# kaiidams/Kokoro-Align

Hardware: NVIDIA B200
Metric: lattice cells/sec (TxS) (higher is better)
Workload: dtype f32

## Files before the change

kokoro-align_b200/csrc/kab_api.cu:

```cuda
#include "../../include/kokoro_align_b200.h"

#include <algorithm>
#include <atomic>
#include <chrono>
#include <map>
#include <mutex>
#include <thread>
#include <unordered_map>
#include <cstdio>
#include <cstdlib>
#include <cstring>
#include <limits>
#include <new>
#include <vector>

#include "kab_band.cuh"
#include "kab_bandp.cuh"
#include "kab_bandr.cuh"
#include "kab_btpar.cuh"
#include "kab_wide.cuh"
#include "kab_common.cuh"
#include "kab_compact.cuh"
#include "kab_debug.h"
#include "kab_generic.cuh"
// ... 316 lines not shown
      if (mask && !mask[b]) continue;
      const int64_t T = t_off[b + 1] - t_off[b], S = 2 * (l_off[b + 1] - l_off[b]) + 1;
      if (band_shaped(T, S)) { any_band = true; ok = std::min<int64_t>(W, S) <= ga_max_weff; }
    }
    pl->band_ga = ok && any_band;
  }
  if (!ctc && V > MAX_STAGE_V && M <= 4) {
    std::vector<uint8_t> seen((size_t)V, 0);
    int64_t dmax = 0;
    bool any = false;
    for (int64_t b = 0; b < B; ++b) {
      if (mask && !mask[b]) continue;
      const int64_t L = l_off[b + 1] - l_off[b];
      const int32_t *lab = labels + l_off[b];
      if (pl->band_ga && band_shaped(t_off[b + 1] - t_off[b], 2 * L + 1)) continue;
      bool usable = true;
      int64_t dist = 0;
      for (int64_t l = 0; l < L && usable; ++l) {
        if (lab[l] <= 0 || lab[l] >= V) usable = false;
        else if (!seen[(size_t)lab[l]]) { seen[(size_t)lab[l]] = 1; ++dist; }
      }
      for (int64_t l = 0; l < L; ++l)
        if (lab[l] > 0 && lab[l] < V) seen[(size_t)lab[l]] = 0;
      if (usable) { dmax = std::max(dmax, dist); any = true; }
    }
    if (any && dmax + 1 <= MAX_STAGE_V) {
      pl->Vc = (int32_t)std::max<int64_t>(8, align_up(dmax + 1, 4));
      h_gather.assign((size_t)B * pl->Vc, 0);
    }
  }
  const int32_t Veff = pl->Vc ? pl->Vc : V;

  pl->stage_frames = Veff <= 64 ? 16 : 8;
  if (const char *sf = getenv("KAB_STAGE_FRAMES")) {
    const int v = atoi(sf);
    if (v == 8 || v == 16 || v == 32) pl->stage_frames = v;
  }
  pl->stage_bytes = (int32_t)align_up((int64_t)pl->stage_frames * Veff * 4 + 24, 16);

  int wide_capacity = 0;
  {
    const KabWideGeom wgeo = kab_wide_geom(pl->stage_bytes);
    int occ = 0;
    if (wgeo.smem_bytes <= 227 * 1024 &&
        ensure_dyn_smem((const void *)kab_wide_kernel, device, wgeo.smem_bytes) == cudaSuccess &&
        cudaOccupancyMaxActiveBlocksPerMultiprocessor(&occ, kab_wide_kernel, KAB_WD_THREADS, wgeo.smem_bytes) == cudaSuccess)
      wide_capacity = occ * pl->sm_count;
    (void)cudaGetLastError();
  }
  int wide_max_ctas = 0;

  std::vector<uint16_t> col16;
  std::vector<int32_t> status_init((size_t)B, 0);
  int64_t bp_bytes = 0, scr_floats = 0, max_band_weff = 0;
  std::vector<uint8_t> hyb_mask;
  int hyb_k = 0;
  kab_plan_info &info = pl->info;
  info.n_lattices = B; info.device = device; info.total_frames = pl->total_T;
  const int n_mask = (V + 63) / 64;
  struct LatFacts { uint8_t bad, special, compact; int32_t distinct; int64_t col_off; };
  std::vector<LatFacts> facts((size_t)B);
  auto for_lattices = [&](auto &&fn) {
    const unsigned hw = std::thread::hardware_concurrency();
    const int nt = (B >= 2048 && pl->total_L >= 65536 && hw >= 4 && !getenv("KAB_SERIAL_SETUP")) ? (int)std::min<unsigned>(8, hw / 2) : 1;
    auto work = [&](int t) {
      std::vector<int64_t> words((size_t)std::max(n_mask, 1), 0);
      const int64_t b0 = B * t / nt, b1 = B * (t + 1) / nt;
      for (int64_t b = b0; b < b1; ++b)
        if (!mask || mask[b]) fn(b, words.data());
    };
    std::vector<std::thread> th;
    for (int t = 1; t < nt; ++t) th.emplace_back(work, t);
    work(0);
    for (auto &x : th) x.join();
  };
  for_lattices([&](int64_t b, int64_t *distinct_mask) {
    const int64_t T = t_off[b + 1] - t_off[b], L = l_off[b + 1] - l_off[b], S = 2 * L + 1;
    const int32_t *lab = labels + l_off[b];
    LatFacts f{};
    std::fill(distinct_mask, distinct_mask + n_mask, (int64_t)0);
    for (int64_t l = 0; l < L; ++l) {
      if (ctc ? (lab[l] < 0 || lab[l] >= V || lab[l] == blank) : (lab[l] < -V || lab[l] >= V)) { f.bad = 1; break; }
      if (!ctc && lab[l] <= 0) f.special = 1;
      const int32_t c = lab[l] < 0 ? lab[l] + V : lab[l];
      if (!(distinct_mask[c >> 6] >> (c & 63) & 1)) { distinct_mask[c >> 6] |= (int64_t)1 << (c & 63); ++f.distinct; }
    }
    const bool ga = pl->band_ga && !f.special && band_shaped(T, S);
    if (!f.bad && pl->Vc && !f.special && !ga && f.distinct + 1 <= pl->Vc) {
      f.compact = 1;
      int32_t *g = h_gather.data() + (size_t)b * pl->Vc;
      int32_t n = 1;
      for (int w = 0; w < n_mask; ++w)
        for (int64_t m = distinct_mask[w]; m; m &= m - 1) g[n++] = w * 64 + __builtin_ctzll((unsigned long long)m);
    }
    facts[(size_t)b] = f;
  });
  {
    int64_t off = 0;
    for (int64_t b = 0; b < B; ++b) {
      if (mask && !mask[b]) continue;
      facts[(size_t)b].col_off = off;
      if (!facts[(size_t)b].bad) off += align_up(l_off[b + 1] - l_off[b], 8) + 8;
    }
    col16.assign((size_t)off, 0);
  }
  for_lattices([&](int64_t b, int64_t *) {
    const LatFacts &f = facts[(size_t)b];
    if (f.bad) return;
    const int64_t L = l_off[b + 1] - l_off[b];
    const int32_t *lab = labels + l_off[b];
    uint16_t *c = col16.data() + f.col_off;
    if (f.compact) {
      const int32_t *g = h_gather.data() + (size_t)b * pl->Vc;
      const int32_t n = f.distinct + 1;
      for (int64_t l = 0; l < L; ++l) c[l] = (uint16_t)(std::lower_bound(g + 1, g + n, lab[l]) - g);
    } else {
      for (int64_t l = 0; l < L; ++l) c[l] = (uint16_t)(lab[l] < 0 ? lab[l] + V : lab[l]);
    }
  });
  for (int64_t b = 0; b < B; ++b) {
    if (mask && !mask[b]) continue;
    const int64_t T = t_off[b + 1] - t_off[b], L = l_off[b + 1] - l_off[b], S = 2 * L + 1;
    const bool bad = facts[(size_t)b].bad != 0, special = facts[(size_t)b].special != 0;
    const int64_t distinct = facts[(size_t)b].distinct;
    if (bad) {
      status_init[(size_t)b] = KAB_ST_BAD_LABEL;
      pl->any_bad_label = true;
      continue;
    }
    if (ctc) {
      const int32_t *lab = labels + l_off[b];
      int64_t R = 0;
      for (int64_t l = 1; l < L; ++l) R += lab[l] == lab[l - 1];
      if (T < L + R) {
        status_init[(size_t)b] = KAB_ST_DEAD_BAND;
        pl->any_bad_label = true;
        continue;
      }
    }
    KabLattice d{};
    d.t_off = t_off[b];
    d.lab_off = l_off[b];
    d.T = (int32_t)T; d.L = (int32_t)L; d.index = (int32_t)b;
    d.col_off = facts[(size_t)b].col_off;
    const bool ga = pl->band_ga && !special && band_shaped(T, S);

    const bool fast = M <= 4 && !special && (ga || (Veff <= MAX_STAGE_V && (!pl->Vc || distinct + 1 <= pl->Vc)));
    const bool full = W >= S && (S * (T - 1)) / T <= W / 2;
    const int64_t weff = ctc ? S : std::min<int64_t>(W, S);
    int q;
    if (fast && !ga && full && S <= 248) {
      q = Q_WARP;
      d.k = S <= 62 ? 2 : (S <= 124 ? 4 : (S <= 186 ? 6 : 8));
      const int fpw = d.k <= 2 ? 8 : (d.k <= 4 ? 4 : 2);
      d.bp_off = bp_bytes;
      bp_bytes += align_up((T + fpw - 1) / fpw * 128, 256);
    } else if (fast && W >= 1 && S <= 3 * T && weff + 32 <= KAB_BAND_OW * BAND_MAX_WARPS) {
      q = Q_BAND;
      max_band_weff = std::max(max_band_weff, weff);
    } else if (fast && !ga && M == 4 && full && ((S + KAB_BAND_OW - 1) / KAB_BAND_OW + KAB_WD_CW - 1) / KAB_WD_CW + 1 <= wide_capacity) {
      q = Q_WIDE;
      const int nww = (int)((S + KAB_BAND_OW - 1) / KAB_BAND_OW);
      d.k = nww;
      wide_max_ctas = std::max(wide_max_ctas, (nww + KAB_WD_CW - 1) / KAB_WD_CW);
      d.bp_off = bp_bytes;
      bp_bytes += (int64_t)nww * ((T + 7) / 8) * 256;
      d.scr_off = pl->wide_ws_bytes / 4;
      pl->wide_ws_bytes += (int64_t)align_up((int64_t)kab_wide_ws_bytes(nww), 256);
    } else {
      q = Q_GENERIC;
      d.bp_off = bp_bytes;
      bp_bytes += align_up(T * std::max<int64_t>(1, weff), 256);
      d.scr_off = scr_floats;
      scr_floats += align_up(2 * (S + 16), 64);
    }
    pl->lists[q].push_back(d);
    pl->max_T[q] = std::max(pl->max_T[q], (int)T);
    info.n_class[q == Q_WARP ? KAB_CLASS_WARP : (q == Q_GENERIC ? KAB_CLASS_GENERIC : (q == Q_WIDE ? KAB_CLASS_WIDE : KAB_CLASS_BAND))]++;
    const int64_t cells = ctc ? T * S : cells_eval_of(T, S, W);
    info.cells_eval += cells;
    info.cells_nominal += T * S;
    int bbits = 0;
    while ((1 << bbits) < M) ++bbits;
    const int64_t dcols = std::min<int64_t>(V, distinct + 1);
    info.algorithmic_bytes += 4 * dcols * T + (cells * bbits + 7) / 8 + (T * bbits + 7) / 8 + 12 * T;
  }
  if (!pl->lists[Q_BAND].empty()) {
    pl->band_nw = (int32_t)((max_band_weff + 32 + KAB_BAND_OW - 1) / KAB_BAND_OW);
    const int nc = (pl->band_nw + KAB_BP_CW - 1) / KAB_BP_CW;
    const char *cl = getenv("KAB_BAND_CLUSTER");
    int want_nc = cl ? atoi(cl) : -1;
    if (band_mode >= 0) want_nc = band_mode == 0 ? 0 : -1;
    const bool cluster_ok = nc <= 8 && kab_bandp_geom(pl->stage_bytes).smem_bytes <= 227 * 1024;
    const int nwq = (int)((max_band_weff + 32 + KAB_BQ_OW - 1) / KAB_BQ_OW);
    const int ncq = (nwq + KAB_BQ_CW - 1) / KAB_BQ_CW;
    const bool q_ok = ncq <= 8 && kab_bandq_geom(pl->stage_bytes).smem_bytes <= 227 * 1024;
    const int ncr = (nwq + KAB_BR_CW - 1) / KAB_BR_CW;
    const bool r_ok = pl->band_ga || (ncr <= 8 && pl->stage_frames == KAB_BR_F && kab_bandr_geom(pl->stage_bytes).smem_bytes <= 227 * 1024);
    const char *qe = getenv("KAB_BAND_Q");
    const int want_q = band_mode >= 0 ? (band_mode == 0 ? 0 : -1) : (qe ? atoi(qe) : -1);
    const char *re = getenv("KAB_BAND_R");
    const int want_r = band_mode >= 0 ? band_mode : (re ? atoi(re) : -1);
    int64_t n_band = (int64_t)pl->lists[Q_BAND].size();
    double sum_t = 0.0, max_t = 0.0, bt_steps = 0.0;
    for (const KabLattice &d : pl->lists[Q_BAND]) {
      sum_t += d.T; max_t = std::max(max_t, (double)d.T);
      bt_steps += (double)d.T * (double)std::min<int64_t>(W, 2 * (int64_t)d.L + 1);
    }
    const double est_r = std::max(max_t * 70.0, sum_t / std::max(1, pl->sm_count / std::max(1, ncr)) * 90.0) + bt_steps * 0.55e-3;
    const double est_b = std::max(max_t, sum_t / (double)(pl->sm_count * (pl->band_nw <= 16 ? 2 : 1))) * 190.0;
    const bool use_r = pl->band_ga || (r_ok && want_r != 0 && want_nc != 0 && want_q != 0 && (want_r >= 1 || want_nc >= 1 || est_r <= est_b));
    const bool use_q = !use_r && M == 4 && q_ok && want_q != 0 && want_nc != 0 && (want_q >= 1 || n_band <= pl->sm_count / ncq);
    {
      const char *he = getenv("KAB_BAND_HYBRID");
      const int want_h = he ? atoi(he) : -1;
      if (band_mode < 0 && !mask && !use_r && !use_q && r_ok && !pl->band_ga && !pl->Vc && V <= MAX_STAGE_V && want_h != 0 &&
          want_r < 0 && want_q < 0 && want_nc < 0 && n_band >= 2) {
        std::vector<KabLattice> &bl = pl->lists[Q_BAND];
        std::stable_sort(bl.begin(), bl.end(), [](const KabLattice &a, const KabLattice &b2) { return a.T > b2.T; });
        std::vector<double> pre((size_t)n_band + 1, 0.0);
        for (int64_t i = 0; i < n_band; ++i) pre[(size_t)i + 1] = pre[(size_t)i] + bl[(size_t)i].T;
        const int per_sm = pl->band_nw <= 16 ? 2 : 1;
        double best = est_b;
        int best_k = 0;
        int64_t best_m = 0;
        for (int k = 1; k <= pl->sm_count / ncr / 2; ++k) {
          const double sm_left = (double)(pl->sm_count - k * ncr) * per_sm;
          for (int64_t m = k; m < n_band && m <= 16 * (int64_t)k; ++m) {
            const double tr_ = std::max((double)bl[0].T, pre[(size_t)m] / k) * 70.0;
            const double tb_ = std::max((double)bl[(size_t)m].T, (sum_t - pre[(size_t)m]) / sm_left) * 190.0;
            const double ms = std::max(tr_, tb_);
            if (ms < best) { best = ms; best_k = k; best_m = m; }
          }
        }
        if (want_h >= 1 && best_k == 0) { best_k = 1; best_m = 1; }
        if (best_k > 0 && (want_h >= 1 || best < 0.85 * est_b)) {
          hyb_mask.assign((size_t)B, 0);
          for (int64_t i = 0; i < best_m; ++i) hyb_mask[(size_t)bl[(size_t)i].index] = 1;
          bl.erase(bl.begin(), bl.begin() + best_m);
          hyb_k = best_k;
          want_nc = 0;
          pl->band_sm_reserved = best_k * ncr;
          n_band = (int64_t)bl.size();
          pl->max_T[Q_BAND] = bl.empty() ? 0 : bl[0].T;
        }
      }
    }
    if (use_r || use_q) {
      pl->band_q = true;
      pl->band_r = use_r;
      pl->band_cw = use_r ? KAB_BR_CW : KAB_BQ_CW;
      pl->band_nc = use_r ? ncr : ncq;
      const int nwt = pl->band_cw * pl->band_nc;
      for (KabLattice &d : pl->lists[Q_BAND]) {
        d.bp_off = bp_bytes;
        bp_bytes += (int64_t)((d.T + 7) / 8) * 128 * nwt;
        d.scr_off = pl->band_fifo_bytes / 4;
        pl->band_fifo_bytes += (int64_t)align_up((int64_t)kab_bandq_ws_bytes(nwt), 256);
      }
    } else if ([&] {
      if (want_nc < 0 && cluster_ok) {
        const int64_t resident = pl->sm_count / nc;
        want_nc = (int64_t)pl->lists[Q_BAND].size() <= resident ? nc : 0;
      }
      return M == 4 && cluster_ok && want_nc >= 1; }()) {
      pl->band_nc = std::min(8, std::max(nc, want_nc));
      const int nwt = KAB_BP_CW * pl->band_nc;
      for (KabLattice &d : pl->lists[Q_BAND]) {
        d.bp_off = bp_bytes;
        bp_bytes += (int64_t)((d.T + 7) / 8) * 256 * nwt;
        d.scr_off = pl->band_fifo_bytes / 4;
        pl->band_fifo_bytes += (int64_t)align_up((int64_t)kab_bandp_ws_bytes(nwt), 256);
      }
    } else {
      const KabBandGeom geo = kab_band_geom(pl->band_nw, pl->stage_bytes);
      for (KabLattice &d : pl->lists[Q_BAND]) {
        d.bp_off = bp_bytes;
        bp_bytes += align_up((int64_t)d.T * geo.nbp, 256);
      }
    }
  }
  for (int q = 0; q < N_QUEUES; ++q)
    std::stable_sort(pl->lists[q].begin(), pl->lists[q].end(), [&](const KabLattice &a, const KabLattice &b2) {
      if (q == Q_WARP && a.k != b2.k) return a.k > b2.k;
      return a.T > b2.T;
    });

  bool par_bt = !pl->lists[Q_BAND].empty() && pl->band_nc > 0;
  if (par_bt) {
    const char *sb = getenv("KAB_BAND_SERIAL_BT");
    double steps = 0.0, tmax = 0.0;
    for (const KabLattice &d : pl->lists[Q_BAND]) {
      steps += (double)d.T * (double)std::min<int64_t>(W, 2 * (int64_t)d.L + 1);
      tmax = std::max(tmax, (double)d.T);
    }
    par_bt = pl->band_q || (sb ? atoi(sb) == 0 : steps * 0.55e-12 <= 0.6 * tmax * 40e-9);
  }
  if (par_bt) {
    for (const KabLattice &d : pl->lists[Q_BAND]) {
      KabBtMeta m{};
      m.map_off = pl->bt_map_ints;
      m.first_block = pl->bt_blocks;
      m.n_blocks = (d.T + KAB_BT_BLOCK - 1) / KAB_BT_BLOCK;
      m.wl = (int32_t)align_up(std::min<int64_t>(W, 2 * (int64_t)d.L + 1), 32);
      pl->bt_map_ints += (int64_t)m.n_blocks * KAB_BT_NSUB * m.wl;
      pl->bt_blocks += m.n_blocks;
      pl->bt_max_wl = std::max(pl->bt_max_wl, m.wl);
      pl->bt_meta.push_back(m);
    }
// ... 773 lines not shown
```

kokoro-align_b200/csrc/kab_common.cuh:

```cuda
#pragma once
#include <cuda_runtime.h>
#include <stdint.h>

#define KAB_FULL_MASK 0xffffffffu

struct KabLattice {
  int64_t t_off;
  int64_t col_off;
  int64_t lab_off;
  int64_t bp_off;
  int64_t scr_off;
  int32_t T;
  int32_t L;
  int32_t index;
  int32_t k;
};

struct KabParams {
  const float *lp;
  int64_t lp_bytes;
  const uint16_t *col16;
  const int32_t *raw;
  uint8_t *bp;
  float *scratch;
// ... 16 lines not shown
};

__global__ void kab_gate_kernel(const unsigned int *counter, unsigned int target) {
  if (threadIdx.x == 0) {
    unsigned int v;
    for (;;) {
      asm volatile("ld.acquire.gpu.global.u32 %0, [%1];" : "=r"(v) : "l"(counter) : "memory");
      if ((int)(v - target) >= 0) break;
      __nanosleep(500);
    }
  }
}

template <bool MM>
__device__ __forceinline__ float kab_mm(const float cand, const float mask) {
  return MM ? __fadd_rn(cand, mask) : cand;
}

__device__ __forceinline__ float kab_neg_inf() { return __int_as_float(0xff800000); }
__device__ __forceinline__ bool kab_finite(float x) { return fabsf(x) < __int_as_float(0x7f800000); }
__device__ __forceinline__ float kab_poison(float acc, float x) { return fmaf(x, 0.0f, acc); }

__device__ __forceinline__ float kab_poison_ctc(float acc, float x) { return __fadd_rn(acc, x); }
template <bool CTC>
__device__ __forceinline__ float kab_poison_t(float acc, float x) {
  return CTC ? kab_poison_ctc(acc, x) : kab_poison(acc, x);
}
template <bool CTC>
__device__ __forceinline__ float kab_poison_init() { return CTC ? kab_neg_inf() : 0.0f; }
__device__ __forceinline__ float kab_ctc_blank_sel(float x0, float x1, uint32_t &w, const int pos) {
  const bool p1 = x1 > x0;
  w |= (uint32_t)p1 << pos;
  return p1 ? x1 : x0;
}
__device__ __forceinline__ float kab_ctc_label_sel(float x0, float x1, float x2, uint32_t &w, const int pos) {
  const bool p2 = x2 > x1 && x2 > x0;
  const bool p1 = x1 > x0 && x1 > x2;
  w |= ((uint32_t)p2 << 1 | (uint32_t)p1) << pos;
  return p2 ? x2 : (p1 ? x1 : x0);
}

__device__ __forceinline__ uint32_t kab_smem_u32(const void *p) {
  return (uint32_t)__cvta_generic_to_shared(p);
}
__device__ __forceinline__ void kab_mbar_init(uint64_t *bar, uint32_t count) {
  asm volatile("mbarrier.init.shared::cta.b64 [%0], %1;" ::"r"(kab_smem_u32(bar)), "r"(count) : "memory");
}
__device__ __forceinline__ void kab_fence_mbar_init() {
  asm volatile("fence.mbarrier_init.release.cluster;" ::: "memory");
}
__device__ __forceinline__ void kab_mbar_expect_tx(uint64_t *bar, uint32_t bytes) {
  asm volatile("mbarrier.arrive.expect_tx.shared::cta.b64 _, [%0], %1;" ::"r"(kab_smem_u32(bar)), "r"(bytes)
               : "memory");
}
__device__ __forceinline__ bool kab_mbar_try_wait(uint64_t *bar, uint32_t parity) {
  uint32_t ok;
  asm volatile(
      "{\n\t.reg .pred p;\n\t"
      "mbarrier.try_wait.parity.shared::cta.b64 p, [%1], %2;\n\t"
      "selp.u32 %0, 1, 0, p;\n\t}"
      : "=r"(ok)
      : "r"(kab_smem_u32(bar)), "r"(parity)
      : "memory");
  return ok != 0;
}
__device__ __forceinline__ void kab_mbar_wait(uint64_t *bar, uint32_t parity) {
  while (!kab_mbar_try_wait(bar, parity)) {
  }
}
__device__ __forceinline__ void kab_bulk_g2s(void *dst, const void *src, uint32_t bytes, uint64_t *bar) {
  asm volatile("cp.async.bulk.shared::cluster.global.mbarrier::complete_tx::bytes [%0], [%1], %2, [%3];" ::"r"(
                   kab_smem_u32(dst)),
               "l"(src), "r"(bytes), "r"(kab_smem_u32(bar))
               : "memory");
}
__device__ __forceinline__ void kab_bulk_prefetch_l2(const void *src, uint32_t bytes) {
  asm volatile("cp.async.bulk.prefetch.L2.global [%0], %1;" ::"l"(src), "r"(bytes) : "memory");
}
__device__ __forceinline__ void kab_bulk_g2s_hint(void *dst, const void *src, uint32_t bytes, uint64_t *bar,
                                                  uint64_t policy) {
  asm volatile(
      "cp.async.bulk.shared::cluster.global.mbarrier::complete_tx::bytes.L2::cache_hint [%0], [%1], %2, [%3], %4;" ::"r"(
          kab_smem_u32(dst)),
      "l"(src), "r"(bytes), "r"(kab_smem_u32(bar)), "l"(policy)
      : "memory");
}
__device__ __forceinline__ void kab_fence_proxy_async() { asm volatile("fence.proxy.async;" ::: "memory"); }
__device__ __forceinline__ void kab_fence_proxy_async_smem() {
  asm volatile("fence.proxy.async.shared::cta;" ::: "memory");
}

struct KabStageDesc {
  const char *src;
  uint32_t bytes;
  uint32_t skew;
  uint32_t tail_word;
  uint32_t tail_n;
};

__device__ __forceinline__ KabStageDesc kab_stage_desc(const KabParams &p, int64_t t_off, int32_t f0,
                                                       int32_t nf) {
  KabStageDesc d;
  const int64_t b0 = (t_off + f0) * (int64_t)p.V * 4;
  const int64_t b1 = b0 + (int64_t)nf * p.V * 4;
  const int64_t a0 = b0 & ~(int64_t)15;
  int64_t a1 = (b1 + 15) & ~(int64_t)15;
  if (a1 > p.lp_bytes) a1 = b1 & ~(int64_t)15;
  if (a1 < a0) a1 = a0;
  d.src = reinterpret_cast<const char *>(p.lp) + a0;
  d.bytes = (uint32_t)(a1 - a0);
  d.skew = (uint32_t)((b0 - a0) >> 2);
  d.tail_word = d.bytes >> 2;
  d.tail_n = a1 < b1 ? (uint32_t)((b1 - a1) >> 2) : 0u;
  return d;
}

__device__ __forceinline__ void kab_add2(float lo, float hi, float e, float &olo, float &ohi) {
  asm("{\n\t"
      ".reg .b64 u, v, w;\n\t"
      "mov.b64 u, {%2, %3};\n\t"
      "mov.b64 v, {%4, %4};\n\t"
      "add.rn.f32x2 w, u, v;\n\t"
      "mov.b64 {%0, %1}, w;\n\t"
      "}"
      : "=f"(olo), "=f"(ohi)
      : "f"(lo), "f"(hi), "f"(e));
}
__device__ __forceinline__ unsigned long long kab_pack2(float lo, float hi) {
  unsigned long long u;
  asm("mov.b64 %0, {%1, %2};" : "=l"(u) : "f"(lo), "f"(hi));
  return u;
}
__device__ __forceinline__ void kab_add2p(unsigned long long u, float e, float &olo, float &ohi) {
  asm("{\n\t"
      ".reg .b64 v, w;\n\t"
      "mov.b64 v, {%3, %3};\n\t"
      "add.rn.f32x2 w, %2, v;\n\t"
      "mov.b64 {%0, %1}, w;\n\t"
      "}"
      : "=f"(olo), "=f"(ohi)
      : "l"(u), "f"(e));
}
__device__ __forceinline__ void kab_add2v(float lo, float hi, float elo, float ehi, float &olo, float &ohi) {
  asm("{\n\t"
      ".reg .b64 u, v, w;\n\t"
      "mov.b64 u, {%2, %3};\n\t"
      "mov.b64 v, {%4, %5};\n\t"
      "add.rn.f32x2 w, u, v;\n\t"
      "mov.b64 {%0, %1}, w;\n\t"
      "}"
      : "=f"(olo), "=f"(ohi)
      : "f"(lo), "f"(hi), "f"(elo), "f"(ehi));
}
__device__ __forceinline__ int kab_decode_move(uint32_t code, int v) {
#ifndef KAB_SEL_V1
  (void)v;
  return (int)code;
#else
  return ((v & 1) == 0 && code >= 2u) ? 3 : (int)code;
#endif
}
__device__ __forceinline__ float kab_blank_sel(float a0, float a1, float a3, uint32_t &w, const uint32_t bit1,
                                               const uint32_t bit2, const uint32_t one) {
  float best;
#ifndef KAB_SEL_V1
  asm("{\n\t"
      ".reg .pred p1, p3;\n\t"
      "max.f32 %0, %2, %3, %4;\n\t"
      "setp.neu.f32 p1, %2, %0;\n\t"
      "setp.neu.and.f32 p3, %3, %0, p1;\n\t"
      "@p1 mad.lo.u32 %1, %7, %5, %1;\n\t"
      "@p3 mad.lo.u32 %1, %7, %6, %1;\n\t"
      "}"
      : "=f"(best), "+r"(w)
      : "f"(a0), "f"(a1), "f"(a3), "r"(bit1), "r"(bit2), "r"(one));
#else
  asm("{\n\t"
      ".reg .f32 m;\n\t"
      ".reg .pred p1, p3;\n\t"
      "max.f32 m, %2, %3;\n\t"
      "setp.gt.f32 p1, %3, %2;\n\t"
      "setp.gt.f32 p3, %4, m;\n\t"
      "max.f32 %0, m, %4;\n\t"
      "@p1 mad.lo.u32 %1, %7, %5, %1;\n\t"
      "@p3 mad.lo.u32 %1, %7, %6, %1;\n\t"
      "}"
      : "=f"(best), "+r"(w)
      : "f"(a0), "f"(a1), "f"(a3), "r"(bit1), "r"(bit2), "r"(one));
#endif
  return best;
}
__device__ __forceinline__ float kab_label_sel(float a0, float a1, float a2, float a3, uint32_t &w,
                                               const uint32_t bit1, const uint32_t bit2, const uint32_t one) {
  float best;
#ifndef KAB_SEL_V1
  asm("{\n\t"
      ".reg .f32 m01, z;\n\t"
      ".reg .pred ph, pl;\n\t"
      "max.f32 m01, %2, %3;\n\t"
      "max.f32 %0, m01, %4, %5;\n\t"
      "setp.neu.f32 ph, m01, %0;\n\t"
      "selp.f32 z, %4, %2, ph;\n\t"
      "setp.neu.f32 pl, z, %0;\n\t"
      "@pl mad.lo.u32 %1, %8, %6, %1;\n\t"
      "@ph mad.lo.u32 %1, %8, %7, %1;\n\t"
      "}"
      : "=f"(best), "+r"(w)
      : "f"(a0), "f"(a1), "f"(a2), "f"(a3), "r"(bit1), "r"(bit2), "r"(one));
#else
  asm("{\n\t"
      ".reg .f32 m01, m23, z;\n\t"
      ".reg .pred ph, pl;\n\t"
      "max.f32 m01, %2, %3;\n\t"
      "max.f32 m23, %4, %5;\n\t"
      "setp.gt.f32 ph, m23, m01;\n\t"
      "selp.f32 %0, m23, m01, ph;\n\t"
      "selp.f32 z, %4, %2, ph;\n\t"
      "setp.gt.f32 pl, %0, z;\n\t"
      "@pl mad.lo.u32 %1, %8, %6, %1;\n\t"
      "@ph mad.lo.u32 %1, %8, %7, %1;\n\t"
      "}"
      : "=f"(best), "+r"(w)
      : "f"(a0), "f"(a1), "f"(a2), "f"(a3), "r"(bit1), "r"(bit2), "r"(one));
#endif
  return best;
}
```

kokoro-align_b200/csrc/kab_warp.cuh:

```cuda
#pragma once
#include "kab_common.cuh"

#define KAB_WARP_STAGES 3
#define KAB_WARPS_PER_CTA 4
#ifndef KAB_WARP_MINBLOCKS
#define KAB_WARP_MINBLOCKS 5
#endif

template <int K>
struct KabWarpCfg {
  static constexpr int BPF = K <= 2 ? 4 : (K <= 4 ? 8 : 16);
  static constexpr int FPW = 32 / BPF;
};

template <int K, bool MM>
__device__ __forceinline__ void kab_warp_frame(float (&s)[K], const float eb, const float (&el)[K / 2],
                                               const bool lane1, uint32_t &w, const int shift,
                                               const uint32_t one, const float mm1, const float mm2, const float mm3) {
  float h1, h2, h3;
  if (K >= 4) {
    h1 = __shfl_up_sync(KAB_FULL_MASK, s[K - 1], 1);
    h2 = __shfl_up_sync(KAB_FULL_MASK, s[K - 2], 1);
    h3 = __shfl_up_sync(KAB_FULL_MASK, s[K >= 4 ? K - 3 : 0], 1);
  } else {
    h1 = __shfl_up_sync(KAB_FULL_MASK, s[1], 1);
    h2 = __shfl_up_sync(KAB_FULL_MASK, s[0], 1);
    h3 = __shfl_up_sync(KAB_FULL_MASK, s[1], 2);
    h3 = lane1 ? kab_neg_inf() : h3;
  }
  float t[K];
#pragma unroll
  for (int m = 0; m < K / 2; ++m) kab_add2(s[2 * m], s[2 * m + 1], eb, t[2 * m], t[2 * m + 1]);
  const float th1 = __fadd_rn(h1, eb), th3 = __fadd_rn(h3, eb);
  float n[K];
#pragma unroll
  for (int q = 0; q < K / 2; ++q) {
    const int kb = 2 * q, kl = 2 * q + 1;
    const float b1 = kb >= 1 ? t[kb >= 1 ? kb - 1 : 0] : th1;
    const float b3 = kb >= 3 ? t[kb >= 3 ? kb - 3 : 0] : (kb == 2 ? th1 : th3);
    n[kb] = kab_blank_sel(t[kb], kab_mm<MM>(b1, mm1), kab_mm<MM>(b3, mm3), w, 1u << (shift + 2 * kb), 2u << (shift + 2 * kb), one);
    float a0, a1, a2, a3;
    kab_add2(s[kl - 1], s[kl], el[q], a1, a0);
    if (q >= 1) kab_add2(s[q >= 1 ? kl - 3 : 0], s[q >= 1 ? kl - 2 : 0], el[q], a3, a2);
    else kab_add2(h2, h1, el[q], a3, a2);
    n[kl] = kab_label_sel(a0, kab_mm<MM>(a1, mm1), kab_mm<MM>(a2, mm2), kab_mm<MM>(a3, mm3), w, 1u << (shift + 2 * kl), 2u << (shift + 2 * kl), one);
  }
#pragma unroll
  for (int k = 0; k < K; ++k) s[k] = n[k];
}

template <int K>
__device__ __forceinline__ void kab_warp_frame_ctc(float (&s)[K], const float eb, const float (&el)[K / 2],
                                                   const uint32_t rep, uint32_t &w, const int shift) {
  const float h1 = __shfl_up_sync(KAB_FULL_MASK, s[K - 1], 1);
  float n[K];
#pragma unroll
  for (int q = 0; q < K / 2; ++q) {
    const int kb = 2 * q, kl = 2 * q + 1;
    n[kb] = __fadd_rn(kab_ctc_blank_sel(s[kb], kb >= 1 ? s[kb >= 1 ? kb - 1 : 0] : h1, w, shift + 2 * kb), eb);
    const float x2 = (rep >> q) & 1u ? kab_neg_inf() : (kl >= 3 ? s[kl >= 3 ? kl - 2 : 0] : h1);
    n[kl] = __fadd_rn(kab_ctc_label_sel(s[kl], s[kl - 1], x2, w, shift + 2 * kl), el[q]);
  }
#pragma unroll
  for (int k = 0; k < K; ++k) s[k] = n[k];
}

template <int K, int VCT, bool MM, bool CTC>
__device__ void kab_warp_align(const KabLattice &lat, const KabParams &p, float *stage_base, uint64_t *bars,
                               uint16_t *labtab, const uint64_t policy, uint32_t &chunk_counter, const int lane,
                               const int blank) {
  using Cfg = KabWarpCfg<K>;
  constexpr int BPF = Cfg::BPF, FPW = Cfg::FPW;
  const int T = lat.T, S = 2 * lat.L + 1;
  const int V = VCT ? VCT : p.V;
  const int F = p.stage_frames;
  const uint32_t stage_words = p.stage_bytes >> 2;
  const int n_chunks = (T + F - 1) / F;
  const uint16_t *col16 = p.col16 + lat.col_off;
  uint32_t *bpw = reinterpret_cast<uint32_t *>(p.bp + lat.bp_off);
  const bool lane0 = lane == 0, lane1 = lane == 1;
  const uint32_t one = p.one;
  const float mm1 = p.mm1, mm2 = p.mm2, mm3 = p.mm3;
  const int sbase = K * (lane - 1);

  uint32_t coff[K / 2];
  uint32_t rep = 0;
#pragma unroll
  for (int q = 0; q < K / 2; ++q) {
    const int v = sbase + 2 * q + 1;
    const uint32_t col = (v > 0 && v < S) ? col16[(v - 1) >> 1] : 0u;
    coff[q] = 4u * col;
    if (v > 0 && v < S) labtab[(v - 1) >> 1] = (uint16_t)col;
    if (CTC && (v < 3 || v >= S || col == col16[(v - 3) >> 1])) rep |= 1u << q;
  }
  const uint32_t boff = CTC ? 4u * (uint32_t)blank : 0u;

  float s[K];
#pragma unroll
  for (int k = 0; k < K; ++k) s[k] = kab_neg_inf();
  if (lane1) s[0] = 0.0f;

  const uint32_t cc0 = chunk_counter;
  const int64_t lat_b0 = lat.t_off * (int64_t)V * 4;
  const char *lp_base = reinterpret_cast<const char *>(p.lp) + (lat_b0 & ~(int64_t)15);
  const int w0 = (int)((lat_b0 & 15) >> 2);
  const uint32_t chunk_stride = (uint32_t)(F * V * 4);
  const uint32_t full_bytes = (chunk_stride + (uint32_t)w0 * 4u + 15u) & ~15u;
  uint32_t ist = cc0 % KAB_WARP_STAGES;
  auto issue = [&](int c) {
    float *dst = stage_base + ist * stage_words;
    if (c + 1 < n_chunks) {
      if (lane0) {
        kab_mbar_expect_tx(&bars[ist], full_bytes);
        kab_bulk_g2s_hint(dst, lp_base + (size_t)c * chunk_stride, full_bytes, &bars[ist], policy);
      }
    } else {
      const int f0 = c * F;
      const KabStageDesc d = kab_stage_desc(p, lat.t_off, f0, T - f0);
      if (lane0) {
        kab_mbar_expect_tx(&bars[ist], d.bytes);
        if (d.bytes) kab_bulk_g2s_hint(dst, d.src, d.bytes, &bars[ist], policy);
      }
      if (lane < (int)d.tail_n)
        dst[d.tail_word + lane] = __ldg(reinterpret_cast<const float *>(d.src) + d.tail_word + lane);
    }
    ist = ist + 1 == KAB_WARP_STAGES ? 0 : ist + 1;
  };
  const int pre = min(n_chunks, KAB_WARP_STAGES - 1);
  for (int c = 0; c < pre; ++c) issue(c);

  float poison = kab_poison_init<CTC>();
  uint32_t *bprow = bpw + lane;
  uint32_t st = cc0 % KAB_WARP_STAGES, ph = (cc0 / KAB_WARP_STAGES) & 1u;
  for (int c = 0; c < n_chunks; ++c) {
    __syncwarp();
    if (c + KAB_WARP_STAGES - 1 < n_chunks) issue(c + KAB_WARP_STAGES - 1);
    kab_mbar_wait(&bars[st], ph);
    __syncwarp();
    const int nf = min(F, T - c * F);
    const float *stage = stage_base + st * stage_words;
    if (++st == KAB_WARP_STAGES) { st = 0; ph ^= 1u; }
    const int w1 = w0 + nf * V;
    {
      const int v0 = (w0 + 3) >> 2, v1 = w1 >> 2;
      const float4 *s4 = reinterpret_cast<const float4 *>(stage);
      for (int j = v0 + lane; j < v1; j += 32) {
        const float4 x = s4[j];
        poison = kab_poison_t<CTC>(kab_poison_t<CTC>(kab_poison_t<CTC>(kab_poison_t<CTC>(poison, x.x), x.y), x.z), x.w);
      }
      if (lane < 4 * v0 - w0 && w0 + lane < w1) poison = kab_poison_t<CTC>(poison, stage[w0 + lane]);
      if (4 * v1 >= w0 && lane < w1 - 4 * v1) poison = kab_poison_t<CTC>(poison, stage[4 * v1 + lane]);
    }
    const char *rowb = reinterpret_cast<const char *>(stage + w0);
    const int n_groups = nf / FPW;
    for (int gi = 0; gi < n_groups; ++gi, rowb += FPW * V * 4) {
      uint32_t word = 0;
#pragma unroll
      for (int f = 0; f < FPW; ++f) {
        const char *rb = rowb + f * V * 4;
        const float eb = *reinterpret_cast<const float *>(rb + boff);
        float el[K / 2];
#pragma unroll
        for (int q = 0; q < K / 2; ++q) el[q] = *reinterpret_cast<const float *>(rb + coff[q]);
        if (CTC) kab_warp_frame_ctc<K>(s, eb, el, rep, word, f * BPF);
        else kab_warp_frame<K, MM>(s, eb, el, lane1, word, f * BPF, one, mm1, mm2, mm3);
      }
      *bprow = word;
      bprow += 32;
    }
    const int rem = nf - n_groups * FPW;
    if (rem) {
      uint32_t word = 0;
#pragma unroll 1
      for (int f = 0; f < rem; ++f, rowb += V * 4) {
        const float eb = *reinterpret_cast<const float *>(rowb + boff);
        float el[K / 2];
#pragma unroll
        for (int q = 0; q < K / 2; ++q) el[q] = *reinterpret_cast<const float *>(rowb + coff[q]);
        uint32_t fw = 0;
        if (CTC) kab_warp_frame_ctc<K>(s, eb, el, rep, fw, 0);
        else kab_warp_frame<K, MM>(s, eb, el, lane1, fw, 0, one, mm1, mm2, mm3);
        word |= fw << (f * BPF);
      }
      *bprow = word;
    }
  }
  chunk_counter = cc0 + n_chunks;
  __syncwarp();

  auto score_of = [&](int u) {
    float mine = s[0];
#pragma unroll
    for (int k = 1; k < K; ++k) if (k == u % K) mine = s[k];
    return __shfl_sync(KAB_FULL_MASK, mine, u / K + 1);
  };
  int v;
  if (CTC) {
    v = S - 1;
    if (S >= 2) {
      const float a1 = score_of(S - 1), a2 = score_of(S - 2);
      if (!(a1 > a2)) v = S - 2;
    }
  } else {
    int cand = -1;
#pragma unroll
    for (int k = 0; k < K; ++k) {
      const int v = sbase + k;
      if (v >= 0 && v < S && s[k] > kab_neg_inf()) cand = v;
    }
    v = __reduce_max_sync(KAB_FULL_MASK, cand);
  }
  const bool any_bad = __any_sync(KAB_FULL_MASK, poison != poison);
  const int status = any_bad ? 3 : (v < 0 ? 1 : 0);
  {
    float fs = __int_as_float(0x7fc00000);
    if (status == 0) {
      float mine = s[0];
#pragma unroll
      for (int k = 1; k < K; ++k) if (k == v % K) mine = s[k];
      fs = __shfl_sync(KAB_FULL_MASK, mine, v / K + 1);
    }
    if (lane0) {
      p.status[lat.index] = status;
      if (p.final_score) p.final_score[lat.index] = fs;
    }
  }
  if (status != 0) return;

  constexpr int RB = 4;
  int32_t *out_path = p.best_path + lat.t_off;
  int32_t *out_lab = p.best_labels + lat.t_off;
  float *out_sc = p.best_scores + lat.t_off;
  const float *lp = p.lp + lat.t_off * (int64_t)V;
  const int n_rows = (T + FPW - 1) / FPW;
  auto fetch = [&](int rb, uint32_t (&w)[RB]) {
#pragma unroll
    for (int r = 0; r < RB; ++r)
      w[r] = (rb >= 0 && (rb + r) < n_rows) ? __ldcg(&bpw[(size_t)(rb + r) * 32 + lane]) : 0u;
  };
  int myv = 0, pend_t = -1;
  float pend_s = 0.0f;
  int own1 = v / K + 1, k2 = 2 * (v - (v / K) * K);
  uint32_t wr[RB], wn[RB];
  const int rb_last = ((n_rows - 1) / RB) * RB;
  fetch(rb_last, wr);
  for (int rb = rb_last; rb >= 0; rb -= RB) {
    fetch(rb - RB, wn);
    const int fb = rb * FPW;
    const int lb = lane - (fb & 31);
#pragma unroll
    for (int r = RB - 1; r >= 0; --r) {
#pragma unroll
      for (int f = FPW - 1; f >= 0; --f) {
        const uint32_t w = __shfl_sync(KAB_FULL_MASK, wr[r], own1);
        if (lb == r * FPW + f) myv = v;
        const int mv = (int)((w >> (f * BPF + k2)) & 3u);
        v -= mv;
        k2 -= 2 * mv;
        if (k2 < 0) { k2 += 2 * K; --own1; }
        if (K == 2 && k2 < 0) { k2 += 2 * K; --own1; }
      }
    }
    if ((fb & 31) == 0) {
      if (pend_t >= 0) out_sc[pend_t] = pend_s;
      const int t = fb + lane;
      pend_t = -1;
      if (t < T) {
        const int lab = (myv & 1) ? (int)labtab[(myv - 1) >> 1] : (CTC ? blank : 0);
        out_path[t] = myv;
        out_lab[t] = lab;
        pend_s = __ldg(&lp[(int64_t)t * V + lab]);
        pend_t = t;
      }
    }
#pragma unroll
    for (int r = 0; r < RB; ++r) wr[r] = wn[r];
  }
  if (pend_t >= 0) out_sc[pend_t] = pend_s;
}

template <int VCT, bool MM, bool CTC>
__device__ __forceinline__ void kab_warp_body(const KabLattice *__restrict__ lats, int n_lat, const KabParams &p,
                                              const int blank) {
  extern __shared__ __align__(128) unsigned char kab_smem[];
  const int warp = threadIdx.x >> 5, lane = threadIdx.x & 31;
  uint64_t *bars = reinterpret_cast<uint64_t *>(kab_smem) + warp * KAB_WARP_STAGES;
  float *stage_base = reinterpret_cast<float *>(kab_smem + 128 +
                                                (size_t)warp * KAB_WARP_STAGES * p.stage_bytes);
  uint16_t *labtab = reinterpret_cast<uint16_t *>(kab_smem + 128 +
                                                  (size_t)KAB_WARPS_PER_CTA * KAB_WARP_STAGES * p.stage_bytes) +
                     warp * 128;
  uint64_t policy;
  asm volatile("createpolicy.fractional.L2::evict_normal.b64 %0, 1.0;" : "=l"(policy));
  if (lane == 0) {
    for (int s = 0; s < KAB_WARP_STAGES; ++s) kab_mbar_init(&bars[s], 1);
    kab_fence_mbar_init();
  }
  __syncwarp();
  uint32_t chunk_counter = 0;
  for (;;) {
    unsigned int item = 0;
    if (lane == 0) item = atomicAdd(p.queue, 1u);
    item = __shfl_sync(KAB_FULL_MASK, item, 0);
    if (item >= (unsigned int)n_lat) break;
    const KabLattice lat = lats[item];
    switch (lat.k) {
      case 2: kab_warp_align<2, VCT, MM, CTC>(lat, p, stage_base, bars, labtab, policy, chunk_counter, lane, blank); break;
      case 4: kab_warp_align<4, VCT, MM, CTC>(lat, p, stage_base, bars, labtab, policy, chunk_counter, lane, blank); break;
      case 6: kab_warp_align<6, VCT, MM, CTC>(lat, p, stage_base, bars, labtab, policy, chunk_counter, lane, blank); break;
      default: kab_warp_align<8, VCT, MM, CTC>(lat, p, stage_base, bars, labtab, policy, chunk_counter, lane, blank); break;
    }
    __syncwarp();
  }
}

template <int VCT, bool MM>
__global__ void __launch_bounds__(KAB_WARPS_PER_CTA * 32, KAB_WARP_MINBLOCKS)
    kab_warp_kernel(const KabLattice *__restrict__ lats, int n_lat, KabParams p) {
  kab_warp_body<VCT, MM, false>(lats, n_lat, p, 0);
}

__global__ void __launch_bounds__(KAB_WARPS_PER_CTA * 32, KAB_WARP_MINBLOCKS)
    kab_warp_ctc_kernel(const KabLattice *__restrict__ lats, int n_lat, KabParams p, int blank) {
  kab_warp_body<0, false, true>(lats, n_lat, p, blank);
}
```

Baseline: 1516 billion.

## Replace backpointer storage with score checkpoints and windowed recompute for wide warp lattices

For non-CTC warp-path lattices with K>=6, the forward pass no longer records 2-bit backpointers per cell. It computes max-only transitions and stores full score rows every C=8 frames as checkpoints. The backtrace streams the emission chunks again in reverse and recomputes each 8-frame block inside a 3C-wide window around the current state to rebuild the moves. This cuts forward-pass selection and bit-packing work but adds a second pass over the emissions and more checkpoint memory traffic. Min blocks per SM is also raised from 5 to 6.

After: 1725 billion, median of 6. +13.7%, better.

```diff
diff --git a/kokoro-align_b200/csrc/kab_api.cu b/kokoro-align_b200/csrc/kab_api.cu
--- a/kokoro-align_b200/csrc/kab_api.cu
+++ b/kokoro-align_b200/csrc/kab_api.cu
@@ -492,9 +492,13 @@
     if (fast && !ga && full && S <= 248) {
       q = Q_WARP;
       d.k = S <= 62 ? 2 : (S <= 124 ? 4 : (S <= 186 ? 6 : 8));
-      const int fpw = d.k <= 2 ? 8 : (d.k <= 4 ? 4 : 2);
       d.bp_off = bp_bytes;
-      bp_bytes += align_up((T + fpw - 1) / fpw * 128, 256);
+      if (ctc || d.k <= 4) {
+        const int fpw = d.k <= 2 ? 8 : (d.k <= 4 ? 4 : 2);
+        bp_bytes += align_up((T + fpw - 1) / fpw * 128, 256);
+      } else {
+        bp_bytes += align_up((T + KAB_CKPT_C - 1) / KAB_CKPT_C * kab_ckpt_stride((int)S, d.k) * 4, 256);
+      }
     } else if (fast && W >= 1 && S <= 3 * T && weff + 32 <= KAB_BAND_OW * BAND_MAX_WARPS) {
       q = Q_BAND;
       max_band_weff = std::max(max_band_weff, weff);
diff --git a/kokoro-align_b200/csrc/kab_common.cuh b/kokoro-align_b200/csrc/kab_common.cuh
--- a/kokoro-align_b200/csrc/kab_common.cuh
+++ b/kokoro-align_b200/csrc/kab_common.cuh
@@ -192,6 +192,16 @@
       : "=f"(olo), "=f"(ohi)
       : "f"(lo), "f"(hi), "f"(elo), "f"(ehi));
 }
+__device__ __forceinline__ float kab_max2(float a, float b) {
+  float m;
+  asm("max.f32 %0, %1, %2;" : "=f"(m) : "f"(a), "f"(b));
+  return m;
+}
+__device__ __forceinline__ float kab_max3(float a, float b, float c) {
+  float m;
+  asm("max.f32 %0, %1, %2, %3;" : "=f"(m) : "f"(a), "f"(b), "f"(c));
+  return m;
+}
 __device__ __forceinline__ int kab_decode_move(uint32_t code, int v) {
 #ifndef KAB_SEL_V1
   (void)v;
diff --git a/kokoro-align_b200/csrc/kab_warp.cuh b/kokoro-align_b200/csrc/kab_warp.cuh
--- a/kokoro-align_b200/csrc/kab_warp.cuh
+++ b/kokoro-align_b200/csrc/kab_warp.cuh
@@ -4,8 +4,12 @@
 #define KAB_WARP_STAGES 3
 #define KAB_WARPS_PER_CTA 4
 #ifndef KAB_WARP_MINBLOCKS
-#define KAB_WARP_MINBLOCKS 5
+#define KAB_WARP_MINBLOCKS 6
 #endif
+
+#define KAB_CKPT_C 8
+
+__host__ __device__ inline int kab_ckpt_stride(int S, int K) { return (K * ((S + K - 1) / K) + 3) & ~3; }
 
 template <int K>
 struct KabWarpCfg {
@@ -15,8 +19,7 @@
 
 template <int K, bool MM>
 __device__ __forceinline__ void kab_warp_frame(float (&s)[K], const float eb, const float (&el)[K / 2],
-                                               const bool lane1, uint32_t &w, const int shift,
-                                               const uint32_t one, const float mm1, const float mm2, const float mm3) {
+                                               const bool lane1, const float mm1, const float mm2, const float mm3) {
   float h1, h2, h3;
   if (K >= 4) {
     h1 = __shfl_up_sync(KAB_FULL_MASK, s[K - 1], 1);
@@ -28,6 +31,37 @@
     h3 = __shfl_up_sync(KAB_FULL_MASK, s[1], 2);
     h3 = lane1 ? kab_neg_inf() : h3;
   }
+  float n[K];
+#pragma unroll
+  for (int q = 0; q < K / 2; ++q) {
+    const int kb = 2 * q, kl = 2 * q + 1;
+    const float b1 = kb >= 1 ? s[kb >= 1 ? kb - 1 : 0] : h1;
+    const float b3 = kb >= 3 ? s[kb >= 3 ? kb - 3 : 0] : (kb == 2 ? h1 : h3);
+    const float mb = kab_max3(s[kb], kab_mm<MM>(b1, mm1), kab_mm<MM>(b3, mm3));
+    const float l2 = q >= 1 ? s[q >= 1 ? kl - 2 : 0] : h1;
+    const float l3 = q >= 1 ? s[q >= 1 ? kl - 3 : 0] : h2;
+    const float ml = kab_max3(kab_max2(s[kl], kab_mm<MM>(s[kl - 1], mm1)), kab_mm<MM>(l2, mm2), kab_mm<MM>(l3, mm3));
+    kab_add2v(mb, ml, eb, el[q], n[kb], n[kl]);
+  }
+#pragma unroll
+  for (int k = 0; k < K; ++k) s[k] = n[k];
+}
+
+template <int K, bool MM>
+__device__ __forceinline__ void kab_warp_frame_bp(float (&s)[K], const float eb, const float (&el)[K / 2],
+                                               const bool lane1, uint32_t &w, const int shift,
+                                                  const uint32_t one, const float mm1, const float mm2, const float mm3) {
+  float h1, h2, h3;
+  if (K >= 4) {
+    h1 = __shfl_up_sync(KAB_FULL_MASK, s[K - 1], 1);
+    h2 = __shfl_up_sync(KAB_FULL_MASK, s[K - 2], 1);
+    h3 = __shfl_up_sync(KAB_FULL_MASK, s[K >= 4 ? K - 3 : 0], 1);
+  } else {
+    h1 = __shfl_up_sync(KAB_FULL_MASK, s[1], 1);
+    h2 = __shfl_up_sync(KAB_FULL_MASK, s[0], 1);
+    h3 = __shfl_up_sync(KAB_FULL_MASK, s[1], 2);
+    h3 = lane1 ? kab_neg_inf() : h3;
+  }
   float t[K];
 #pragma unroll
   for (int m = 0; m < K / 2; ++m) kab_add2(s[2 * m], s[2 * m + 1], eb, t[2 * m], t[2 * m + 1]);
@@ -50,6 +84,18 @@
 }
 
 template <int K>
+__device__ __forceinline__ void kab_ckpt_store(float *row, const float (&s)[K]) {
+  if (K % 4 == 0) {
+#pragma unroll
+    for (int k = 0; k < K; k += 4)
+      __stcg(reinterpret_cast<float4 *>(row + k), make_float4(s[k], s[k + 1], s[k + 2], s[k + 3]));
+  } else {
+#pragma unroll
+    for (int k = 0; k < K; k += 2) __stcg(reinterpret_cast<float2 *>(row + k), make_float2(s[k], s[k + 1]));
+  }
+}
+
+template <int K>
 __device__ __forceinline__ void kab_warp_frame_ctc(float (&s)[K], const float eb, const float (&el)[K / 2],
                                                    const uint32_t rep, uint32_t &w, const int shift) {
   const float h1 = __shfl_up_sync(KAB_FULL_MASK, s[K - 1], 1);
@@ -71,6 +117,8 @@
                                const int blank) {
   using Cfg = KabWarpCfg<K>;
   constexpr int BPF = Cfg::BPF, FPW = Cfg::FPW;
+  constexpr int C = KAB_CKPT_C;
+  constexpr bool BP = CTC || K <= 4;
   const int T = lat.T, S = 2 * lat.L + 1;
   const int V = VCT ? VCT : p.V;
   const int F = p.stage_frames;
@@ -78,6 +126,8 @@
   const int n_chunks = (T + F - 1) / F;
   const uint16_t *col16 = p.col16 + lat.col_off;
   uint32_t *bpw = reinterpret_cast<uint32_t *>(p.bp + lat.bp_off);
+  float *ck = reinterpret_cast<float *>(p.bp + lat.bp_off);
+  const int RS = kab_ckpt_stride(S, K);
   const bool lane0 = lane == 0, lane1 = lane == 1;
   const uint32_t one = p.one;
   const float mm1 = p.mm1, mm2 = p.mm2, mm3 = p.mm3;
@@ -131,6 +181,7 @@
 
   float poison = kab_poison_init<CTC>();
   uint32_t *bprow = bpw + lane;
+  float *ckrow = ck;
   uint32_t st = cc0 % KAB_WARP_STAGES, ph = (cc0 / KAB_WARP_STAGES) & 1u;
   for (int c = 0; c < n_chunks; ++c) {
     __syncwarp();
@@ -152,37 +203,63 @@
       if (4 * v1 >= w0 && lane < w1 - 4 * v1) poison = kab_poison_t<CTC>(poison, stage[4 * v1 + lane]);
     }
     const char *rowb = reinterpret_cast<const char *>(stage + w0);
-    const int n_groups = nf / FPW;
-    for (int gi = 0; gi < n_groups; ++gi, rowb += FPW * V * 4) {
-      uint32_t word = 0;
-#pragma unroll
-      for (int f = 0; f < FPW; ++f) {
-        const char *rb = rowb + f * V * 4;
-        const float eb = *reinterpret_cast<const float *>(rb + boff);
-        float el[K / 2];
-#pragma unroll
-        for (int q = 0; q < K / 2; ++q) el[q] = *reinterpret_cast<const float *>(rb + coff[q]);
-        if (CTC) kab_warp_frame_ctc<K>(s, eb, el, rep, word, f * BPF);
-        else kab_warp_frame<K, MM>(s, eb, el, lane1, word, f * BPF, one, mm1, mm2, mm3);
-      }
-      *bprow = word;
-      bprow += 32;
-    }
-    const int rem = nf - n_groups * FPW;
-    if (rem) {
-      uint32_t word = 0;
+    if constexpr (BP) {
+      const int n_groups = nf / FPW;
+      for (int gi = 0; gi < n_groups; ++gi, rowb += FPW * V * 4) {
+        uint32_t word = 0;
+#pragma unroll
+        for (int f = 0; f < FPW; ++f) {
+          const char *rb = rowb + f * V * 4;
+          const float eb = *reinterpret_cast<const float *>(rb + boff);
+          float el[K / 2];
+#pragma unroll
+          for (int q = 0; q < K / 2; ++q) el[q] = *reinterpret_cast<const float *>(rb + coff[q]);
+          if (CTC) kab_warp_frame_ctc<K>(s, eb, el, rep, word, f * BPF);
+          else kab_warp_frame_bp<K, MM>(s, eb, el, lane1, word, f * BPF, one, mm1, mm2, mm3);
+        }
+        *bprow = word;
+        bprow += 32;
+      }
+      const int rem = nf - n_groups * FPW;
+      if (rem) {
+        uint32_t word = 0;
+#pragma unroll 1
+        for (int f = 0; f < rem; ++f, rowb += V * 4) {
+          const float eb = *reinterpret_cast<const float *>(rowb + boff);
+          float el[K / 2];
+#pragma unroll
+          for (int q = 0; q < K / 2; ++q) el[q] = *reinterpret_cast<const float *>(rowb + coff[q]);
+          uint32_t fw = 0;
+          if (CTC) kab_warp_frame_ctc<K>(s, eb, el, rep, fw, 0);
+          else kab_warp_frame_bp<K, MM>(s, eb, el, lane1, fw, 0, one, mm1, mm2, mm3);
+          word |= fw << (f * BPF);
+        }
+        *bprow = word;
+      }
+    } else {
+      const int n_groups = nf / C;
+      for (int gi = 0; gi < n_groups; ++gi, rowb += C * V * 4) {
+#pragma unroll
+        for (int f = 0; f < C; ++f) {
+          const char *rb = rowb + f * V * 4;
+          const float eb = *reinterpret_cast<const float *>(rb);
+          float el[K / 2];
+#pragma unroll
+          for (int q = 0; q < K / 2; ++q) el[q] = *reinterpret_cast<const float *>(rb + coff[q]);
+          kab_warp_frame<K, MM>(s, eb, el, lane1, mm1, mm2, mm3);
+        }
+        if (!lane0 && sbase < S) kab_ckpt_store<K>(ckrow + sbase, s);
+        ckrow += RS;
+      }
+      const int rem = nf - n_groups * C;
 #pragma unroll 1
       for (int f = 0; f < rem; ++f, rowb += V * 4) {
-        const float eb = *reinterpret_cast<const float *>(rowb + boff);
+        const float eb = *reinterpret_cast<const float *>(rowb);
         float el[K / 2];
 #pragma unroll
         for (int q = 0; q < K / 2; ++q) el[q] = *reinterpret_cast<const float *>(rowb + coff[q]);
-        uint32_t fw = 0;
-        if (CTC) kab_warp_frame_ctc<K>(s, eb, el, rep, fw, 0);
-        else kab_warp_frame<K, MM>(s, eb, el, lane1, fw, 0, one, mm1, mm2, mm3);
-        word |= fw << (f * BPF);
-      }
-      *bprow = word;
+        kab_warp_frame<K, MM>(s, eb, el, lane1, mm1, mm2, mm3);
+      }
     }
   }
   chunk_counter = cc0 + n_chunks;
@@ -226,57 +303,128 @@
     }
   }
   if (status != 0) return;
-
-  constexpr int RB = 4;
-  int32_t *out_path = p.best_path + lat.t_off;
-  int32_t *out_lab = p.best_labels + lat.t_off;
-  float *out_sc = p.best_scores + lat.t_off;
-  const float *lp = p.lp + lat.t_off * (int64_t)V;
-  const int n_rows = (T + FPW - 1) / FPW;
-  auto fetch = [&](int rb, uint32_t (&w)[RB]) {
-#pragma unroll
-    for (int r = 0; r < RB; ++r)
-      w[r] = (rb >= 0 && (rb + r) < n_rows) ? __ldcg(&bpw[(size_t)(rb + r) * 32 + lane]) : 0u;
-  };
-  int myv = 0, pend_t = -1;
-  float pend_s = 0.0f;
-  int own1 = v / K + 1, k2 = 2 * (v - (v / K) * K);
-  uint32_t wr[RB], wn[RB];
-  const int rb_last = ((n_rows - 1) / RB) * RB;
-  fetch(rb_last, wr);
-  for (int rb = rb_last; rb >= 0; rb -= RB) {
-    fetch(rb - RB, wn);
-    const int fb = rb * FPW;
-    const int lb = lane - (fb & 31);
-#pragma unroll
-    for (int r = RB - 1; r >= 0; --r) {
-#pragma unroll
-      for (int f = FPW - 1; f >= 0; --f) {
-        const uint32_t w = __shfl_sync(KAB_FULL_MASK, wr[r], own1);
-        if (lb == r * FPW + f) myv = v;
-        const int mv = (int)((w >> (f * BPF + k2)) & 3u);
-        v -= mv;
-        k2 -= 2 * mv;
-        if (k2 < 0) { k2 += 2 * K; --own1; }
-        if (K == 2 && k2 < 0) { k2 += 2 * K; --own1; }
-      }
-    }
-    if ((fb & 31) == 0) {
-      if (pend_t >= 0) out_sc[pend_t] = pend_s;
-      const int t = fb + lane;
-      pend_t = -1;
-      if (t < T) {
-        const int lab = (myv & 1) ? (int)labtab[(myv - 1) >> 1] : (CTC ? blank : 0);
-        out_path[t] = myv;
-        out_lab[t] = lab;
-        pend_s = __ldg(&lp[(int64_t)t * V + lab]);
-        pend_t = t;
-      }
-    }
-#pragma unroll
-    for (int r = 0; r < RB; ++r) wr[r] = wn[r];
-  }
-  if (pend_t >= 0) out_sc[pend_t] = pend_s;
+  if constexpr (!BP) {
+    int32_t *out_path = p.best_path + lat.t_off;
+    int32_t *out_lab = p.best_labels + lat.t_off;
+    float *out_sc = p.best_scores + lat.t_off;
+    int ve = v;
+    auto win_load = [&](int row, int sb, float &r0, float &r1) {
+      const float *rp = ck + (size_t)max(row, 0) * RS;
+      r0 = __ldcg(rp + max(sb + lane, 0));
+      r1 = __ldcg(rp + max(sb + 32 + lane, 0));
+    };
+    int sb = ve - 63;
+    float r0, r1;
+    win_load((T - 1) / C - 1, sb, r0, r1);
+    for (int k = 0; k < pre; ++k) issue(n_chunks - 1 - k);
+    for (int k = 0; k < n_chunks; ++k) {
+      const int c = n_chunks - 1 - k;
+      __syncwarp();
+      if (k + KAB_WARP_STAGES - 1 < n_chunks) issue(c - (KAB_WARP_STAGES - 1));
+      kab_mbar_wait(&bars[st], ph);
+      __syncwarp();
+      const int nf = min(F, T - c * F);
+      const char *rows = reinterpret_cast<const char *>(stage_base + st * stage_words + w0);
+      if (++st == KAB_WARP_STAGES) { st = 0; ph ^= 1u; }
+      for (int bi = (nf - 1) / C; bi >= 0; --bi) {
+        const int f0 = c * F + bi * C, n = min(C, nf - bi * C);
+        const char *rb = rows + bi * C * V * 4;
+        const int base = ve - 3 * C;
+        const int wi = base + lane - sb;
+        const float x0 = __shfl_sync(KAB_FULL_MASK, r0, wi & 31), x1 = __shfl_sync(KAB_FULL_MASK, r1, wi & 31);
+        const int u = base + lane;
+        float x = u < 0 ? kab_neg_inf() : (wi >= 32 ? x1 : x0);
+        if (f0 == 0) x = u == 0 ? 0.0f : kab_neg_inf();
+        sb = ve - 63;
+        win_load(f0 / C - 2, sb, r0, r1);
+        const bool blank_lane = (u & 1) == 0;
+        const uint32_t uoff = (u > 0 && u < S && !blank_lane) ? 4u * labtab[(u - 1) >> 1] : 0u;
+        uint32_t cw = 0;
+#pragma unroll
+        for (int j = 0; j < C; ++j) {
+          const float e = *reinterpret_cast<const float *>(rb + j * V * 4 + uoff);
+          const float h1 = __shfl_up_sync(KAB_FULL_MASK, x, 1);
+          const float h2 = __shfl_up_sync(KAB_FULL_MASK, x, 2);
+          const float h3 = __shfl_up_sync(KAB_FULL_MASK, x, 3);
+          float a0, a1, a2, a3;
+          kab_add2(x, h1, e, a0, a1);
+          kab_add2(h2, h3, e, a2, a3);
+          a2 = blank_lane ? kab_neg_inf() : kab_mm<MM>(a2, mm2);
+          x = kab_label_sel(a0, kab_mm<MM>(a1, mm1), a2, kab_mm<MM>(a3, mm3), cw, 1u << (2 * j), 2u << (2 * j), one);
+        }
+        if (n < C) cw &= (1u << (2 * n)) - 1u;
+        int wl = 3 * C;
+        uint32_t mw = 0;
+#pragma unroll
+        for (int j = C - 1; j >= 0; --j) {
+          const uint32_t w = __shfl_sync(KAB_FULL_MASK, cw, wl);
+          mw |= w & (3u << (2 * j));
+          wl -= (int)((w >> (2 * j)) & 3u);
+        }
+        const uint32_t above = mw >> min(2 * lane + 2, 2 * C);
+        const int myv = ve - (__popc(above & 0x55555555u) + 2 * __popc(above & 0xaaaaaaaau));
+        ve = base + wl;
+        if (lane < n) {
+          const int lab = (myv & 1) ? (int)labtab[(myv - 1) >> 1] : 0;
+          out_path[f0 + lane] = myv;
+          out_lab[f0 + lane] = lab;
+          out_sc[f0 + lane] = *reinterpret_cast<const float *>(rb + lane * V * 4 + lab * 4);
+        }
+      }
+    }
+    chunk_counter += n_chunks;
+  } else {
+    constexpr int RB = 4;
+    int32_t *out_path = p.best_path + lat.t_off;
+    int32_t *out_lab = p.best_labels + lat.t_off;
+    float *out_sc = p.best_scores + lat.t_off;
+    const float *lp = p.lp + lat.t_off * (int64_t)V;
+    const int n_rows = (T + FPW - 1) / FPW;
+    auto fetch = [&](int rb, uint32_t (&w)[RB]) {
+#pragma unroll
+      for (int r = 0; r < RB; ++r)
+        w[r] = (rb >= 0 && (rb + r) < n_rows) ? __ldcg(&bpw[(size_t)(rb + r) * 32 + lane]) : 0u;
+    };
+    int myv = 0, pend_t = -1;
+    float pend_s = 0.0f;
+    int own1 = v / K + 1, k2 = 2 * (v - (v / K) * K);
+    uint32_t wr[RB], wn[RB];
+    const int rb_last = ((n_rows - 1) / RB) * RB;
+    fetch(rb_last, wr);
+    for (int rb = rb_last; rb >= 0; rb -= RB) {
+      fetch(rb - RB, wn);
+      const int fb = rb * FPW;
+      const int lb = lane - (fb & 31);
+#pragma unroll
+      for (int r = RB - 1; r >= 0; --r) {
+#pragma unroll
+        for (int f = FPW - 1; f >= 0; --f) {
+          const uint32_t w = __shfl_sync(KAB_FULL_MASK, wr[r], own1);
+          if (lb == r * FPW + f) myv = v;
+          const int mv = (int)((w >> (f * BPF + k2)) & 3u);
+          v -= mv;
+          k2 -= 2 * mv;
+          if (k2 < 0) { k2 += 2 * K; --own1; }
+          if (K == 2 && k2 < 0) { k2 += 2 * K; --own1; }
+        }
+      }
+      if ((fb & 31) == 0) {
+        if (pend_t >= 0) out_sc[pend_t] = pend_s;
+        const int t = fb + lane;
+        pend_t = -1;
+        if (t < T) {
+          const int lab = (myv & 1) ? (int)labtab[(myv - 1) >> 1] : (CTC ? blank : 0);
+          out_path[t] = myv;
+          out_lab[t] = lab;
+          pend_s = __ldg(&lp[(int64_t)t * V + lab]);
+          pend_t = t;
+        }
+      }
+#pragma unroll
+      for (int r = 0; r < RB; ++r) wr[r] = wn[r];
+    }
+    if (pend_t >= 0) out_sc[pend_t] = pend_s;
+  }
 }
 
 template <int VCT, bool MM, bool CTC>
```
